# jinhan/tacotron2-vae

Measured on AMD Instinct MI355X. Metric: mel-frames/s (train step, batch=6, 80-mel), higher is better.
Workload: dtype f32; 1 GPU; configs[1]: Tacotron2-VAE fp32 train step (fwd+loss+bwd+clip+Adam), B=6/GPU fixed shape T_in=84 T_out=400, dropout on, random-init seed 1234; step_mode=hip-graph replay, decoder_forward=persistent, decoder_backward=persistent, startup_steps=43, global_batch=6, parallelism=dp1

## Files before the change

include/t2vae.h:

```cpp
#ifndef T2VAE_H
#define T2VAE_H
#include <stdint.h>
#ifdef __cplusplus
extern "C" {
#endif

#define T2V_OK 0
#define T2V_ERR_DIMS -1
#define T2V_ERR_ARG -2
#define T2V_ERR_LAUNCH -3

const char* t2v_version(void);
const char* t2v_last_error(void);

void t2v_set_phase_profile(unsigned long long* dev_buf32);
int t2v_stamp(unsigned long long* dev_buf, int slot, void* stream);
int t2v_debug_spin(int wgs, int microseconds, void* stream);

typedef struct t2v_step_params {
    uint64_t epoch;
    float lr;
    float bc1;
    float bc2s;
    float kl_weight;
// ... 223 lines not shown

int t2v_bn_act_fwd(const float* y, const float* stat_part, int nblk, const float* gamma, const float* beta,
                   float* running_mean, float* running_var, float* mean_out, float* rstd_out, float* out,
                   int B, int M, int T, int act, int training, float p_drop, float momentum, float eps,
                   uint64_t seed, uint32_t rng_stream, uint32_t rng_t, void* stream);
int t2v_bn_act_fwd_len(const float* y, const float* gamma, const float* beta, const float* running_mean,
                       const float* running_var, float* out, const int32_t* lengths, int B, int M, int T, int act, float eps,
                       void* stream);
int t2v_bn_act_bwd(const float* y, const float* dout, const float* mean, const float* rstd,
                   const float* gamma, const float* beta, float* dy, float* dgamma, float* dbeta,
                   float* dconv_bias, int B, int M, int T, int act, float p_drop, uint64_t seed,
                   uint32_t rng_stream, uint32_t rng_t, void* stream);
int t2v_bn_act_bwd_eval(const float* y, const float* dout, const float* mean, const float* rstd,
                   const float* gamma, const float* beta, float* dy, float* dgamma, float* dbeta,
                   float* dconv_bias, int B, int M, int T, int act, float p_drop, uint64_t seed,
                   uint32_t rng_stream, uint32_t rng_t, void* stream);

int t2v_embedding_fwd(const long long* ids, const float* W, float* out_bct, int B, int T, int C, int n_symbols, void* stream);
int t2v_embedding_bwd(const long long* ids, const float* dy_bct, float* dW, int B, int T, int C, int n_symbols, void* stream);

int t2v_gemm_epilogue_bwd(const float* dy, const float* y, float* out, size_t n, float scale, void* stream);

long t2v_colsum_scratch_floats(long M, long N);
int t2v_colsum(const float* A, long lda, long M, long N, float* scratch, float* out, void* stream);

int t2v_mask_outputs(float* mel, float* mel_post, float* gate, const int* lengths, int B, int C, int T, float gate_fill,
                     void* stream);
int t2v_mask_time(const float* x, float* out, const int32_t* lengths, int B, int C, int T, void* stream);
int t2v_reparam_fwd(const float* eps, const float* mu, const float* logvar, float* z, long n, void* stream);
int t2v_reparam_bwd(const float* dz, const float* eps, const float* logvar, float* dlogvar, long n, void* stream);
int t2v_gather_words(const void* const* src, void* const* dst, int n, void* stream);
int t2v_concat2_rows(const float* a, long lda, int na, const float* b, long ldb, int nb, float* out, long rows, void* stream);

int t2v_bilstm_fwd(const float* gx, const float* whh, const int32_t* lengths, float* y, float* gates,
                   float* cells, float* hx_scratch, uint32_t* sync3, int B, int T, void* stream);
int t2v_bilstm_bwd(const float* whh, const int32_t* lengths, const float* dy, const float* gates,
                   const float* cells, float* dg, float* dgx_scratch, uint32_t* sync3, int B, int T,
                   void* stream);

int t2v_gemm_f32(const float* A, long sAi, long sAk, const float* B, long sBj, long sBk, const float* bias,
                 float* C, int ldc, int M, int N, int K, int relu, int accumulate, float p_drop,
                 uint64_t seed, uint32_t rng_stream, uint32_t rng_t, void* stream);
long t2v_gemm_splitk_scratch_floats(int M, int N, int K);
int t2v_gemm_f32_splitk(const float* A, long sAi, long sAk, const float* B, long sBj, long sBk, const float* bias,
                        float* C, int ldc, int M, int N, int K, int relu, int accumulate, float p_drop,
                        uint64_t seed, uint32_t rng_stream, uint32_t rng_t, float* splitk_scratch, void* stream);

int t2v_gemm_f32_set_mode(int x3);

typedef struct t2v_gemm_group {
    const float* A;
    long sAi;
    long sAk;
    int nb;
    const float* B[3];
    long sBj[3];
    long sBk[3];
    int N[3];
    float* C[3];
    int ldc[3];
} t2v_gemm_group;
long t2v_gemm_f32_grouped_scratch_floats(const t2v_gemm_group* groups, int ngroups, int M, int K);
int t2v_gemm_f32_grouped(const t2v_gemm_group* groups, int ngroups, int M, int K, int accumulate, float* scratch, void* stream);
long t2v_gemm_f32_grouped_group_offset(const t2v_gemm_group* groups, int ngroups, int M, int K, int g);
int t2v_gemm_f32_grouped_handed(const t2v_gemm_group* groups, int ngroups, int M, int K, int accumulate, float* scratch, int handed,
                                const uint32_t* done_ctr, int done_cap, void* stream);
// ... 160 lines not shown
```

tacotron2-vae_amd/csrc/gemm.hip:

```cpp
#include <stdlib.h>
#include <string.h>
#include "t2v_common.h"
#include "t2v_kernels.h"
#include "t2v_coop.h"
#include "t2v_x3.h"
#include "t2v_xchg.h"
#include "gemm_x3_tile.h"

#define GM_BM 64
#define GM_BN 64
#define GM_BK 32

struct GemmArgs {
    const float* A; const float* B; const float* bias; float* C;
    long sAi, sAk, sBj, sBk;
    int M, N, K, ldc;
    int relu, accumulate;
    float p_drop; uint64_t seed; uint32_t rng_stream, rng_t;
    const t2v_step_params* step;
    int kz_chunk;
    float* part;
    int nbatch;
    long sAb, sBb, sCb;
    int nsub;
// ... 137 lines not shown
                || hipDeviceSynchronize() != hipSuccess) { state.store(0); return nullptr; }
            ring = p;
            state.store(2, std::memory_order_release);
        } else {
            while (state.load(std::memory_order_acquire) == 1) { }
            if (state.load() != 2) return nullptr;
        }
    }
    unsigned at = pos.fetch_add((unsigned)tiles);
    at %= GM_CTR_RING;
    if (at + (unsigned)tiles > GM_CTR_RING) {
        pos.store((unsigned)tiles);
        at = 0;
    }
    return ring + at;
}
static int gemm_splits(int M, int N, int K) {
    const long tiles = (long)((M + GM_BM - 1) / GM_BM) * ((N + GM_BN - 1) / GM_BN);
    static const int wide = getenv("T2V_GEMM_SPLIT_POLICY") ? atoi(getenv("T2V_GEMM_SPLIT_POLICY")) : 1;
    if (wide) {
        if (tiles > 256 || K < 8 * GM_BK) return 1;
        long ns2 = (512 + tiles - 1) / tiles;
        const long maxk2 = K / (4 * GM_BK);
        if (ns2 > maxk2) ns2 = maxk2;
        if (ns2 > 32) ns2 = 32;
        return ns2 < 2 ? 1 : (int)ns2;
    }
    if (tiles >= 256 || K < 16 * GM_BK) return 1;
    long ns = 512 / tiles;
    const long maxk = K / (8 * GM_BK);
    if (ns > maxk) ns = maxk;
    if (ns > 32) ns = 32;
    return ns < 2 ? 1 : (int)ns;
}
static bool gemm_x3_shape_ok(int M, int N, int K);
static long gemm_x3_scratch_floats(int M, int N, int K, int np);
static int gemm_x3_mode();
extern "C" long t2v_gemm_splitk_scratch_floats(int M, int N, int K) {
    if (M < 1 || N < 1 || K < 1) return 0;
    if (gemm_x3_mode() && gemm_x3_shape_ok(M, N, K)) return gemm_x3_scratch_floats(M, N, K, 3);
    const int ns = gemm_splits(M, N, K);
    return ns > 1 ? (long)ns * M * N : 0;
}

#define GB_BM 128
#define GB_BK 32
#define GB_LD 160
template <bool A_KC, bool B_KC, int BN>
__global__ __launch_bounds__(256) void k_gemm_f32_big(GemmArgs a) {
    constexpr int NY = BN / 64;
    constexpr int NA = GB_BM * GB_BK / 4 / 256;
    constexpr int NB = BN * GB_BK / 4 / 256;
    constexpr int KQ = GB_BK / 4;
    __shared__ __attribute__((aligned(16))) float As[2][GB_BK][GB_LD];
    __shared__ __attribute__((aligned(16))) float Bs[2][GB_BK][BN + 32];
    const int tid = threadIdx.x, wave = tid >> 6, lane = tid & 63;
    const int wm = wave >> 1, wn = wave & 1;
    int by_ = blockIdx.y, bx_ = blockIdx.x;
    {
        const int nb = gridDim.x * gridDim.y, bid = blockIdx.y * gridDim.x + blockIdx.x;
        const int q = nb >> 3, r = nb & 7, xcd = bid & 7, idx = bid >> 3;
        const int lin = (xcd < r ? xcd * (q + 1) : r * (q + 1) + (xcd - r) * q) + idx;
        by_ = lin / gridDim.x;
        bx_ = lin - by_ * gridDim.x;
    }
    const int i0 = by_ * GB_BM, j0 = bx_ * BN;
// ... 796 lines not shown
```

tacotron2-vae_amd/csrc/t2v_kernels.h:

```cpp
#pragma once
#include <hip/hip_runtime.h>
#include <stdint.h>
#include <initializer_list>
#include "../../include/t2vae.h"
#include "t2v_common.h"

enum { T2V_RNG_ATT_H = 1, T2V_RNG_ATT_C = 2, T2V_RNG_DEC_H = 3, T2V_RNG_DEC_C = 4,
       T2V_RNG_PRENET0 = 5, T2V_RNG_PRENET1 = 6 };

int t2v_check_launch();
unsigned* t2v_arrival_counters(int n);
extern unsigned long long* g_t2v_prof;
const t2v_step_params* t2v_step_for(hipStream_t stream);

struct T2VZeroRegions {
    void* p[10];
    size_t bytes[10];
    int n = 0;
    void add(void* ptr, size_t nbytes) { p[n] = ptr; bytes[n] = nbytes; ++n; }
};
void t2v_zero_regions(T2VZeroRegions& z, hipStream_t stream);

__global__ void k_sentinel_fill(uint4* p, size_t n16);
void t2v_fill_sentinel(void* p, size_t n16, int grid, hipStream_t stream);
bool t2v_persist_cus_ok();
bool t2v_persist_raise_lds(std::initializer_list<const void*> kernels, bool& raised);
int t2v_persist_resident(const void* kernel, int threads, size_t lds, std::initializer_list<const void*> kernels, bool& raised);
struct LstmFwdArgs;
struct AttnFwdArgs;

typedef unsigned long long t2v_u64;
static inline size_t t2v_tcap(int T_in) { return (size_t)((T_in + 15) / 16) * 16; }
static inline size_t t2v_qp_sync_off(int B) { return (size_t)B * 256 * 128; }
static inline size_t t2v_qp_xchg_off(int B) { return t2v_qp_sync_off(B) + 64; }
static inline size_t t2v_qp_ex_off(int B) { return t2v_qp_sync_off(B) + 64 + 4096; }
#define T2V_MAX_T_IN 4096
static inline size_t t2v_qp_floats(int B, int T_in) { return t2v_qp_ex_off(B) + 2 * (size_t)B * 8 * t2v_tcap(T_in); }
static inline int t2v_attn_bwd_js(int T_in) { return T_in <= 128 ? 16 : 32; }
static inline int t2v_attn_bwd_slices_(int T_in) { const int js = t2v_attn_bwd_js(T_in); return (T_in + js - 1) / js; }
void t2v_launch_lstm_fwd(int mode, const LstmFwdArgs& a, hipStream_t stream);
void t2v_launch_attn_fwd(const AttnFwdArgs& f, int B, int T_in, hipStream_t stream);
void t2v_launch_attn_fwd_window(const AttnFwdArgs& f, int B, int T_in, int back, int ahead, hipStream_t stream);
static inline unsigned* t2v_persist_fwd_begin(const t2v_dec_train_persist_weights* w, const t2v_dec_train_bufs* s, const float* scratch,
                                              int B, int T_in, hipStream_t stream) {
// ... 129 lines not shown
```

tacotron2-vae_amd/model.py:

```python
from math import sqrt

import os

import torch
from torch import nn
from torch.nn import functional as F

import t2v_hip
from layers import ConvNorm, LinearNorm
from modules import VAE_GST
from utils import get_mask_from_lengths, to_gpu

drop_rate = 0.5
_drop_seed = [0x5EED]


class LocationLayer(nn.Module):
    def __init__(self, attention_n_filters, attention_kernel_size, attention_dim):
        super().__init__()
        self.location_conv = ConvNorm(2, attention_n_filters, kernel_size=attention_kernel_size,
                                      padding=(attention_kernel_size - 1) // 2, bias=False, stride=1,
                                      dilation=1)
        self.location_dense = LinearNorm(attention_n_filters, attention_dim, bias=False, w_init_gain='tanh')

# ... 335 lines not shown
        dec = self.decoder_rnn
        return (dec.bias_ih + dec.bias_hh,
                torch.cat((self.linear_projection.weight, self.gate_layer.weight), 0),
                torch.cat((self.linear_projection.bias, self.gate_layer.bias), 0))

    def forward(self, memory, decoder_inputs, memory_lengths):
        B, T_in = memory.size(0), memory.size(1)
        prep = self.__dict__.pop('_prepared', None)
        gpre = None
        operands = None
        if prep is not None and prep[0] is decoder_inputs:
            _, pre, gpre, st, operands = prep
            T = pre.size(0)
            if st != torch.cuda.current_stream():
                torch.cuda.current_stream().wait_stream(st)
                for t in operands:
                    t.record_stream(torch.cuda.current_stream())
        else:
            frames = self.parse_decoder_inputs(decoder_inputs)
            T = frames.size(0)
            x = torch.cat((self.get_go_frame(memory).unsqueeze(0), frames), 0)
            pre = self.prenet(x[:T], self._tf_rng_t())
        att = self.attention_rnn
        lin = t2v_hip.LinearHIP.apply
        pm = lin(memory, self.attention_layer.memory_layer.weight, None, False, 0.0, 0, 0, 0)
        lengths = lengths_i32(memory_lengths, memory.device)
        training = self.training
        p_att = self.p_attention_dropout if training else 0.0
        p_dec = self.p_decoder_dropout if training else 0.0
        self._calls += 1
        seed = (int(self.dropout_seed) * 1000003 + self._calls) & 0x7FFFFFFFFFFFFFFF
        t2v_hip.stamp('dec_fwd_begin')
        b_dec, w81, b81 = operands if operands is not None else self._param_operands()
        hc, alignments = t2v_hip.DecoderCore.apply(None, memory, pm, lengths, *self._core_weights(b_dec),
                                                   p_att, p_dec, seed, torch.is_grad_enabled(),
                                                   pre, att.bias_ih, att.bias_hh, gpre)
        t2v_hip.stamp('dec_fwd_end')
        out = lin(hc, w81, b81, False, 0.0, 0, 0, 0)
        mel = out[..., :self.n_mel_channels].permute(1, 2, 0).contiguous()
        gate = out[..., self.n_mel_channels].transpose(0, 1).contiguous()
        return mel, gate, alignments


class SymbolEmbedding(nn.Embedding):

    def forward(self, ids):
        return t2v_hip.SymbolEmbedding.apply(ids, self.weight)


def lengths_i32(lengths, device):
    v = getattr(lengths, '_i32', None)
    if v is not None and v.device == device:
        return v
    return lengths.to(device=device, dtype=torch.int32)


class BatchLayout(object):
    _DT = (torch.int64, torch.int64, torch.float32, torch.float32, torch.int64, torch.float32, torch.float32)
    _ring = {}
    RING = 4
    n_symbols = None

    @classmethod
    def check_ids(cls, text):
        if cls.n_symbols is not None and text.numel() and not text.is_cuda:
            lo, hi = int(text.min()), int(text.max())
            if lo < 0 or hi >= cls.n_symbols:
                raise IndexError("symbol id out of range: got [%d, %d], embedding has %d rows" % (lo, hi, cls.n_symbols))

# ... 160 lines not shown
```

tacotron2-vae_amd/t2v_hip.py:

```python
import collections
import ctypes as C
import math
import operator
import os

import torch

_HERE = os.path.dirname(os.path.abspath(__file__))
_LIB_PATH = os.environ.get('T2V_LIB') or os.path.join(_HERE, 'libt2vae_hip.so')
_lib = None

H, E, PRE, A, F_LOC, KS, XW, KATT, KATT_INF, G4 = 1024, 512, 256, 128, 32, 31, 2560, 1536, 1792, 4096


class T2VHipError(RuntimeError):
    pass


class _DecWeights(C.Structure):
    _fields_ = [(n, C.c_void_p) for n in (
        'packF_att', 'packF_dec', 'packB_att', 'packB_dec', 'bias_att', 'bias_dec', 'wqT', 'wcomb', 'v')] + [
        ('packs_bf16', C.c_int32)]


# ... 52 lines not shown
    _fields_ = [('back', C.c_int32), ('ahead', C.c_int32)]


EXPORTS = ('t2v_version', 't2v_last_error', 't2v_stamp', 't2v_debug_spin', 't2v_pack_lstm_weights', 't2v_pack_lstm_weights_bf16', 't2v_decoder_train_fwd',
           't2v_decoder_train_bwd', 't2v_clip_adam_step', 't2v_clip_adam_step_guarded', 't2v_decoder_replay_fwd_kernels', 't2v_mel_frontend', 't2v_set_phase_profile', 't2v_decoder_infer_steps', 't2v_conv1d_stat_blocks', 't2v_conv1d_stat_blocks_bf16', 't2v_conv1d_staged_launches', 't2v_conv1d_fwd', 't2v_conv1d_bwd', 't2v_conv1d_fwd_bf16', 't2v_conv1d_bwd_bf16', 't2v_conv1d_dw_scratch_floats', 't2v_conv1d_flip_weights', 't2v_gemm_bf16', 't2v_gemm_bf16_splitk', 't2v_gemm_bf16_splitk_scratch_floats', 't2v_attn_wgrad', 't2v_attn_wgrad_scratch_floats',
           't2v_bn_act_fwd', 't2v_bn_act_bwd', 't2v_bn_act_bwd_eval', 't2v_bilstm_fwd', 't2v_bilstm_bwd', 't2v_gemm_f32', 't2v_conv2d_s2_fwd', 't2v_conv2d_s2_bwd', 't2v_conv2d_s2_dw_scratch_floats', 't2v_conv2d_s2_fwd_gemm', 't2v_conv2d_s2_bwd_gemm',
           't2v_conv2d_s2_gemm_scratch_floats',
           't2v_gru_fwd', 't2v_gru_bwd', 't2v_loss_fwd_bwd', 't2v_fuse_location_weights', 't2v_decoder_qp_floats',
           't2v_set_step_params', 't2v_set_step_params_stream', 't2v_decoder_replay_bwd_kernels', 't2v_embedding_fwd', 't2v_embedding_bwd', 't2v_gemm_f32_splitk', 't2v_gemm_splitk_scratch_floats', 't2v_gemm_f32_batched',
           't2v_decoder_infer_persistent', 't2v_decoder_persist_supported', 't2v_decoder_persist_scratch_floats',
           't2v_attn_bwd_slices', 't2v_colsum', 't2v_colsum_scratch_floats', 't2v_gemm_epilogue_bwd',
           't2v_decoder_train_fwd_persistent', 't2v_decoder_train_persist_supported',
           't2v_decoder_train_persist_scratch_floats', 't2v_decoder_bwd_persist_supported',
           't2v_decoder_bwd_achain_scratch_floats', 't2v_decoder_bwd_achain', 't2v_decoder_bwd_achain_prepare',
           't2v_decoder_bwd_achain_prepared', 't2v_decoder_bwd_persist_slices', 't2v_decoder_bwd_achain_dq_offset',
           't2v_decoder_bwd_achain_dw_offset', 't2v_gemm_f32_grouped_handed', 't2v_gemm_f32_grouped_group_offset', 't2v_mask_outputs', 't2v_reparam_fwd',
           't2v_reparam_bwd', 't2v_gather_words', 't2v_concat2_rows',
           't2v_decoder_train_fwd_persistent16', 't2v_decoder_train_persist16_supported',
           't2v_decoder_train_persist16_scratch_floats', 't2v_decoder_bwd_persistent16', 't2v_decoder_bwd_persist16_supported',
           't2v_decoder_bwd_persist16_scratch_floats', 't2v_decoder_bwd_persist16_dq_offset', 't2v_decoder_bwd_persist16_slices',
           't2v_decoder_bwd_persist16_fits', 't2v_gemm_f32_set_mode', 't2v_conv1d_x3_set_mode', 't2v_gemm_f32_grouped',
           't2v_gemm_f32_grouped_scratch_floats', 't2v_gemm_bf16_grouped', 't2v_gemm_bf16_grouped_scratch_floats',
           't2v_decoder_bwd_persistent16_prepare', 't2v_decoder_bwd_persistent16_prepared',
           't2v_stft_polar', 't2v_istft', 't2v_istft_scratch_bytes', 't2v_griffin_lim', 't2v_griffin_lim_scratch_bytes',
           't2v_mel_to_magnitude', 't2v_decoder_infer_steps_items', 't2v_decoder_infer_persistent_items', 't2v_bn_act_fwd_len',
           't2v_mask_time', 't2v_conv2d_s2_fwd_ragged', 't2v_conv2d_s2_fwd_gemm_ragged', 't2v_conv2d_s2_gemm_ragged_scratch_floats',
           't2v_gru_fwd_len', 't2v_mel_dtw', 't2v_mel_dtw_scratch_bytes', 't2v_tsne_scratch_bytes', 't2v_tsne_affinities',
           't2v_tsne_gradient', 't2v_tsne_run', 't2v_f0_yin', 't2v_alignment_stats', 't2v_alignment_scratch_bytes',
           't2v_mel_to_magnitude_nnls', 't2v_griffin_lim_fast', 't2v_griffin_lim_fast_scratch_bytes',
           't2v_resample', 't2v_trim_bounds', 't2v_crop_rows', 't2v_latent_scratch_bytes', 't2v_latent_neighbours',
           't2v_mel_cepstrum', 't2v_cep_dtw_scratch_bytes', 't2v_cep_dtw_path', 't2v_cep_dtw_forward', 't2v_cep_dtw_walk',
           't2v_path_scores', 't2v_loudness', 't2v_loudness_scratch_bytes', 't2v_scale_rows',
           't2v_decoder_infer_steps_window', 't2v_decoder_infer_persistent_window',
           't2v_phase_vocoder', 't2v_phase_vocoder_scratch_bytes')


def lib_path():
    return _LIB_PATH


def load_library():
    global _lib
    if _lib is not None:
        return _lib
    if not os.path.isfile(_LIB_PATH):
        raise T2VHipError("libt2vae_hip.so not built: run `python -c 'import __graft_entry__ as g; g.build()'` "
                          "(or make -C tacotron2-vae_amd/csrc)")
    lib = C.CDLL(_LIB_PATH)
    lib.t2v_version.restype = C.c_char_p
    lib.t2v_last_error.restype = C.c_char_p
    lib.t2v_pack_lstm_weights.argtypes = [C.c_void_p, C.c_void_p, C.c_void_p, C.c_void_p, C.c_int, C.c_void_p,
                                          C.c_void_p, C.c_void_p, C.c_void_p, C.c_void_p]
    lib.t2v_pack_lstm_weights_bf16.argtypes = [C.c_void_p, C.c_void_p, C.c_void_p, C.c_void_p, C.c_int, C.c_void_p,
                                          C.c_void_p, C.c_void_p, C.c_void_p, C.c_void_p]
    lib.t2v_fuse_location_weights.argtypes = [C.c_void_p, C.c_void_p, C.c_void_p, C.c_void_p]
    lib.t2v_decoder_qp_floats.argtypes = [C.c_int, C.c_int]
    lib.t2v_decoder_qp_floats.restype = C.c_long
    lib.t2v_attn_bwd_slices.argtypes = [C.c_int]
    lib.t2v_decoder_train_fwd.argtypes = [C.POINTER(_DecWeights), C.POINTER(_DecTrainBufs), C.c_int, C.c_int,
                                          C.c_int, C.c_float, C.c_float, C.c_uint64, C.c_void_p]
    lib.t2v_decoder_train_bwd.argtypes = [C.POINTER(_DecWeights), C.POINTER(_DecTrainBufs),
                                          C.POINTER(_DecBwdBufs), C.c_int, C.c_int, C.c_int, C.c_float,
                                          C.c_float, C.c_uint64, C.c_void_p]
    lib.t2v_decoder_train_fwd_persistent.argtypes = [C.POINTER(_DecTrainPersistWeights), C.POINTER(_DecTrainBufs), C.c_void_p,
                                                     C.c_int, C.c_int, C.c_int, C.c_float, C.c_float, C.c_uint64, C.c_void_p]
    lib.t2v_decoder_train_persist_supported.argtypes = [C.c_int, C.c_int]
    lib.t2v_decoder_train_fwd_persistent16.argtypes = lib.t2v_decoder_train_fwd_persistent.argtypes
# ... 22 lines not shown
    lib.t2v_decoder_train_persist_scratch_floats.argtypes = [C.c_int, C.c_int, C.c_int]
    lib.t2v_decoder_train_persist_scratch_floats.restype = C.c_long
    lib.t2v_decoder_bwd_persist_supported.argtypes = [C.c_int, C.c_int]
    lib.t2v_decoder_bwd_achain_scratch_floats.argtypes = [C.c_int, C.c_int, C.c_int]
    lib.t2v_decoder_bwd_achain_scratch_floats.restype = C.c_long
    lib.t2v_gemm_f32_grouped_handed.argtypes = [C.POINTER(_GemmGroup), C.c_int, C.c_int, C.c_int, C.c_int, C.c_void_p, C.c_int, C.c_void_p,
                                                C.c_int, C.c_void_p]
    lib.t2v_gemm_f32_grouped_group_offset.argtypes = [C.POINTER(_GemmGroup), C.c_int, C.c_int, C.c_int, C.c_int]
    lib.t2v_gemm_f32_grouped_group_offset.restype = C.c_long
    lib.t2v_decoder_bwd_achain_dw_offset.argtypes = [C.c_int, C.c_int, C.c_int]
    lib.t2v_decoder_bwd_achain_dw_offset.restype = C.c_long
    lib.t2v_decoder_bwd_achain.argtypes = [C.POINTER(_DecTrainPersistWeights), C.POINTER(_AchainDw), C.POINTER(_DecTrainBufs)] + [C.c_void_p] * 8 + [
        C.c_int, C.c_int, C.c_int, C.c_float, C.c_float, C.c_uint64, C.c_void_p]
    lib.t2v_decoder_bwd_persist_slices.argtypes = [C.c_int]
    lib.t2v_decoder_bwd_achain_dq_offset.argtypes = [C.c_int, C.c_int, C.c_int]
    lib.t2v_decoder_bwd_achain_dq_offset.restype = C.c_long
    lib.t2v_decoder_bwd_achain_prepared.argtypes = lib.t2v_decoder_bwd_achain.argtypes
    lib.t2v_decoder_bwd_achain_prepare.argtypes = [C.POINTER(_DecTrainBufs), C.c_void_p, C.c_void_p, C.c_void_p, C.c_int, C.c_int, C.c_int,
                                                   C.c_float, C.c_float, C.c_uint64, C.c_void_p]
    lib.t2v_decoder_replay_fwd_kernels.argtypes = [C.POINTER(_DecWeights), C.POINTER(_DecTrainBufs), C.c_int,
                                                   C.c_int, C.c_int, C.c_float, C.c_float, C.c_uint64, C.c_int,
                                                   C.c_void_p]
    lib.t2v_decoder_replay_bwd_kernels.argtypes = [C.POINTER(_DecWeights), C.POINTER(_DecTrainBufs),
                                                   C.POINTER(_DecBwdBufs), C.c_int, C.c_int, C.c_int, C.c_float,
                                                   C.c_float, C.c_uint64, C.c_int, C.c_void_p]
    lib.t2v_clip_adam_step.argtypes = [C.c_void_p, C.c_void_p, C.c_void_p, C.c_void_p, C.c_uint64, C.c_float,
                                       C.c_float, C.c_float, C.c_float, C.c_float, C.c_float, C.c_float,
                                       C.c_float, C.c_float, C.c_void_p, C.c_void_p, C.c_void_p]
    lib.t2v_clip_adam_step_guarded.argtypes = lib.t2v_clip_adam_step.argtypes[:-1] + [C.c_void_p, C.c_int, C.c_void_p]
    lib.t2v_mask_outputs.argtypes = [C.c_void_p] * 4 + [C.c_int, C.c_int, C.c_int, C.c_float, C.c_void_p]
    lib.t2v_reparam_fwd.argtypes = [C.c_void_p] * 4 + [C.c_long, C.c_void_p]
    lib.t2v_reparam_bwd.argtypes = [C.c_void_p] * 4 + [C.c_long, C.c_void_p]
    lib.t2v_concat2_rows.argtypes = [C.c_void_p, C.c_long, C.c_int, C.c_void_p, C.c_long, C.c_int, C.c_void_p, C.c_long, C.c_void_p]
    lib.t2v_gather_words.argtypes = [C.POINTER(C.c_void_p), C.POINTER(C.c_void_p), C.c_int, C.c_void_p]
    lib.t2v_embedding_fwd.argtypes = [C.c_void_p, C.c_void_p, C.c_void_p, C.c_int, C.c_int, C.c_int, C.c_int, C.c_void_p]
    lib.t2v_embedding_bwd.argtypes = [C.c_void_p, C.c_void_p, C.c_void_p, C.c_int, C.c_int, C.c_int, C.c_int, C.c_void_p]
    lib.t2v_gemm_epilogue_bwd.argtypes = [C.c_void_p, C.c_void_p, C.c_void_p, C.c_size_t, C.c_float, C.c_void_p]
    lib.t2v_colsum.argtypes = [C.c_void_p, C.c_long, C.c_long, C.c_long, C.c_void_p, C.c_void_p, C.c_void_p]
    lib.t2v_colsum_scratch_floats.argtypes = [C.c_long, C.c_long]
    lib.t2v_colsum_scratch_floats.restype = C.c_long
    lib.t2v_set_step_params.argtypes = [C.c_void_p]
    lib.t2v_set_step_params.restype = None
    lib.t2v_set_step_params_stream.argtypes = [C.c_void_p, C.c_void_p]
    lib.t2v_mel_frontend.argtypes = [C.c_void_p, C.c_void_p, C.c_void_p, C.c_int, C.c_int, C.c_float, C.c_int,
                                     C.c_int, C.c_int, C.c_void_p, C.c_void_p, C.c_void_p, C.c_void_p, C.c_void_p,
                                     C.c_void_p, C.c_int, C.c_void_p, C.c_int, C.c_void_p]
    lib.t2v_set_phase_profile.argtypes = [C.c_void_p]
    lib.t2v_set_phase_profile.restype = None
    lib.t2v_stamp.argtypes = [C.c_void_p, C.c_int, C.c_void_p]
    lib.t2v_debug_spin.argtypes = [C.c_int, C.c_int, C.c_void_p]
    lib.t2v_decoder_infer_persistent.argtypes = [C.POINTER(_DecPersistWeights), C.POINTER(_DecPersistBufs), C.c_int, C.c_int,
                                                 C.c_int, C.c_float, C.c_float, C.c_uint64, C.c_void_p]
    lib.t2v_decoder_infer_persistent_items.argtypes = lib.t2v_decoder_infer_persistent.argtypes[:-1] + [C.POINTER(_DecItems),
                                                                                                        C.c_void_p]
    lib.t2v_decoder_persist_supported.argtypes = [C.c_int, C.c_int]
    lib.t2v_decoder_persist_scratch_floats.argtypes = [C.c_int, C.c_int]
    lib.t2v_decoder_persist_scratch_floats.restype = C.c_long
    lib.t2v_decoder_infer_steps.argtypes = [C.POINTER(_DecWeights), C.POINTER(_DecInferBufs), C.c_int, C.c_int, C.c_int,
                                            C.c_int, C.c_float, C.c_float, C.c_int, C.c_uint64, C.c_void_p]
    lib.t2v_decoder_infer_steps_items.argtypes = lib.t2v_decoder_infer_steps.argtypes[:-1] + [C.POINTER(_DecItems), C.c_void_p]
    lib.t2v_decoder_infer_steps_window.argtypes = lib.t2v_decoder_infer_steps_items.argtypes[:-1] + [C.POINTER(_DecWindow), C.c_void_p]
    lib.t2v_decoder_infer_persistent_window.argtypes = lib.t2v_decoder_infer_persistent_items.argtypes[:-1] + [C.POINTER(_DecWindow),
                                                                                                               C.c_void_p]
    vp = C.c_void_p
    lib.t2v_stft_polar.argtypes = [vp, vp, C.c_int, C.c_int, C.c_int, C.c_int, vp, vp, vp, vp, vp, C.c_int, vp]
    lib.t2v_istft_scratch_bytes.argtypes = [C.c_int, C.c_int]
# ... 654 lines not shown
    _check(load_library().t2v_decoder_replay_bwd_kernels(C.byref(W), C.byref(Sb), C.byref(Gb), B, T_in, T, p_att, p_dec,
                                                         seed, int(kernel_mask), _stream()),
           't2v_decoder_replay_bwd_kernels')
    return T if kernel_mask == 1 else T + 1


def pack_decoder_weights(w_ih_att, w_hh_att, w_ih_dec, w_hh_dec, k_att, need_bwd, bf16=False, need_fwd=True):
    lib = load_library()
    dev = w_ih_att.device
    f32 = dict(device=dev, dtype=torch.float32)
    w_ih_att, w_hh_att, w_ih_dec, w_hh_dec = (_f32c(t.detach()) for t in (w_ih_att, w_hh_att, w_ih_dec, w_hh_dec))
    need_fwd = need_fwd or not need_bwd
    packF_att = torch.empty(G4 * k_att, **f32) if need_fwd else None
    packF_dec = torch.empty(G4 * XW, **f32) if need_fwd else None
    packB_att = torch.empty(G4 * KATT, **f32) if need_bwd else None
    packB_dec = torch.empty(G4 * XW, **f32) if need_bwd else None
    fn = lib.t2v_pack_lstm_weights_bf16 if bf16 else lib.t2v_pack_lstm_weights
    _check(fn(_p(w_ih_att), _p(w_hh_att), _p(w_ih_dec), _p(w_hh_dec), int(k_att),
              _p(packF_att), _p(packF_dec), _p(packB_att), _p(packB_dec), _stream()), 't2v_pack_lstm_weights')
    return packF_att, packF_dec, packB_att, packB_dec


def fuse_location_weights(loc_conv, loc_dense):
    lib = load_library()
    wcomb = torch.empty(2, A, 64, device=loc_conv.device, dtype=torch.float32)
    _check(lib.t2v_fuse_location_weights(_p(loc_conv), _p(loc_dense), _p(wcomb), _stream()), 't2v_fuse_location_weights')
    return wcomb


class DecoderCore(torch.autograd.Function):
    persistent = None
    persistent_bwd = None
    persistent16 = None
    keep_last = False
    last_call = None
    last_persist = None
    last_bwd = None
    last_bwd_persist = None
    last_persist_engine = last_bwd_persist_engine = None
    dw_tile_cap = None
    last_mode = None
    last_bwd_mode = None
    last_kernel = None
    last_bwd_kernel = None
    chunk_kernels = []
    chunk_bwd_kernels = []

    @staticmethod
    def plan(lib, B, T_in, T, need_grad):
        D = DecoderCore
        env = os.environ.get
        fwd_on = D.persistent if D.persistent is not None else env('T2V_TRAIN_PERSISTENT', '1') != '0'
        bwd_on = D.persistent_bwd if D.persistent_bwd is not None else env('T2V_BWD_PERSISTENT', env('T2V_TRAIN_PERSISTENT', '1')) != '0'
        on16 = D.persistent16 if D.persistent16 is not None else env('T2V_PERSIST16', '1') != '0'
        force = on16 == 'force'
        on16 = bool(on16) and bool(_BF16)
        small = lambda floats: 4 * floats < 2 ** 31 - 1
        chunks = [(b0, min(B, b0 + MAX_DEC_B)) for b0 in range(0, B, MAX_DEC_B)]
        fwd, bwd = [], []
        for b0, b1 in chunks:
            b = b1 - b0
            p32 = bool(fwd_on) and bool(lib.t2v_decoder_train_persist_supported(b, T_in)) and \
                small(lib.t2v_decoder_train_persist_scratch_floats(b, T_in, T))
            f16 = on16 and bool(fwd_on) and bool(lib.t2v_decoder_train_persist16_supported(b, T_in)) and (force or not p32) and \
                small(lib.t2v_decoder_train_persist16_scratch_floats(b, T_in, T))
            fwd.append('persist16' if f16 else 'persist' if p32 else 'steps')
            if need_grad:
                r32 = bool(bwd_on) and bool(lib.t2v_decoder_bwd_persist_supported(b, T_in)) and \
                    small(lib.t2v_decoder_bwd_achain_scratch_floats(b, T_in, T))
                r16 = on16 and env('T2V_PERSIST16_BWD', '1') != '0' and bool(bwd_on) and \
                    bool(lib.t2v_decoder_bwd_persist16_fits(b, T_in, T)) and (force or not r32)
                bwd.append('persist16' if r16 else 'achain' if r32 else 'steps')
            else:
                bwd.append(None)
        if 'steps' in bwd:
            bwd = ['steps'] * len(bwd)
        dw_on = (not _BF16 and env('T2V_DW_EPILOGUE', '1') != '0' and env('T2V_DW_GROUPED', '1') != '0' and
                 env('T2V_F32_GEMM', '') not in ('native', '0'))
        return [ChunkPlan(b0, b1, f, r, f != 'steps' and r in _BWD_ENGINES, dw_on and r == 'achain')
                for (b0, b1), f, r in zip(chunks, fwd, bwd)]

    @staticmethod
    def _note(fwd=None, bwd=None, **kept):
        D = DecoderCore
        if fwd is not None:
            D.last_mode = 'launch-per-step' if fwd == 'steps' else 'persistent'
            D.last_kernel = _STEPS_KERNELS['fwd'] if fwd == 'steps' else _FWD_ENGINES[fwd].kernel
            D.chunk_kernels.append(D.last_kernel)
        if bwd is not None:
            D.last_bwd_mode = 'launch-per-step' if bwd == 'steps' else 'persistent'
            D.last_bwd_kernel = _STEPS_KERNELS['bwd'] if bwd == 'steps' else _BWD_ENGINES[bwd].kernel
            D.chunk_bwd_kernels.append(D.last_bwd_kernel)
        for name, value in kept.items():
            setattr(D, name, value)

    @staticmethod
    def _wgrad_tensors(ctx, f32):
        if ctx.wg is None:
            wg = [grad_slot(w) for w in ctx.wrefs]
            ctx.wg = [torch.empty(w.shape, **f32) if g is None else g for g, w in zip(wg, ctx.wrefs)]
        return ctx.wg

    @staticmethod
    def _dw_groups(DGA, DGD, XS, wg, pre_c, T, B):
        TB = T * B
        x_prev, x_cur = XS[0:T].reshape(TB, XW), XS[1:T + 1].reshape(TB, XW)
        d_w_ih_att, d_w_hh_att, d_w_ih_dec, d_w_hh_dec = wg
        att = [(x_prev[:, :H].t(), d_w_hh_att), (x_prev[:, H:KATT].t(), d_w_ih_att[:, PRE:])]
        if pre_c is not None:
            att.insert(0, (pre_c.t(), d_w_ih_att[:, :PRE]))
        return [(DGA.view(TB, G4).t(), att), (DGD.view(TB, G4).t(), [(x_cur[:, :KATT].t(), d_w_ih_dec), (x_cur[:, KATT:].t(), d_w_hh_dec)])]

    @staticmethod
# ... 20 lines not shown
        keep = (gpre, memory, pm, lengths, XS, CA, CD, GA, GD, QP, AL, ACUM, S)
        packF_att, packF_dec, packB_att, packB_dec = packs
        W = _DecWeights(_p(packF_att), _p(packF_dec), _p(packB_att), _p(packB_dec), None, _p(bias_dec),
                        _p(wqT), _p(wcomb), _p(vv), int(bool(wbf)))
        Sb = _DecTrainBufs(*(_p(t) for t in keep))
        dims = (B, T_in, T, float(p_att), float(p_dec), int(seed))
        if plan.fwd == 'steps':
            _check(lib.t2v_decoder_train_fwd(C.byref(W), C.byref(Sb), *(dims + (_stream(),))), 't2v_decoder_train_fwd')
            _err_note('decoder forward (attention exchange)', QP.view(torch.int32)[B * 256 * A + 31:][:1])
            DecoderCore._note(fwd='steps')
            return W, Sb, keep, None
        eng = _FWD_ENGINES[plan.fwd]
        scratch = torch.empty(getattr(lib, eng.scratch)(B, T_in, T), **f32)
        PW = _persist_weights(raw, bias_dec, wcomb, vv)
        _check(getattr(lib, eng.run)(C.byref(PW), C.byref(Sb), _p(scratch), *(dims + (_stream(),))), eng.run)
        _err_note('decoder forward (persistent kernel hand-off)', QP.view(torch.int32)[B * 256 * A + 31:][:1])
        DecoderCore._note(fwd=plan.fwd)
        if DecoderCore.keep_last:
            DecoderCore._note(last_persist=(PW, Sb, scratch, dims, raw), last_persist_engine=plan.fwd)
        if not plan.prepare:
            return W, Sb, keep, None
        beng = _BWD_ENGINES[plan.bwd]
        DQP, bscr, errw = DecoderCore._bwd_buffers(lib, beng, B, T_in, T, gpre.device)
        with side('w', keep=tuple(keep[_ARENA.index(n)] for n in beng.keep)):
            args = (_p(DQP), _p(bscr), _p(errw), B, T_in, T)
            if beng.arena_prepare:
                args = (C.byref(Sb),) + args + dims[3:]
            _check(getattr(lib, beng.prepare)(*(args + (_stream(),))), beng.prepare)
            ev = torch.cuda.Event()
            ev.record()
        return W, Sb, keep, (DQP, bscr, errw, ev)

    @staticmethod
    def forward(ctx, gpre, memory, pm, lengths, w_ih_att, w_hh_att, w_ih_dec, w_hh_dec, bias_dec,
                wq, loc_conv, loc_dense, v, p_att, p_dec, seed, grad_mode=True, pre=None, b_ih_att=None, b_hh_att=None,
                gpre_ready=None):
        lib = _require_gpu(memory, pm, w_ih_att)
        pre2 = None
        if pre is not None:
            assert gpre is None
            pre2 = _f32c(pre).view(-1, PRE)
            if gpre_ready is not None:
                gpre = gpre_ready.view(pre.shape[0], pre.shape[1], G4)
            else:
                gpre = gemm(pre2, w_ih_att.detach()[:, :PRE], (b_ih_att + b_hh_att).detach()).view(pre.shape[0], pre.shape[1], G4)
        T, B, _ = gpre.shape
        T_in = memory.shape[1]
        gpre, memory, pm = _f32c(gpre), _f32c(memory), _f32c(pm)
        need_grad = bool(grad_mode) and any(ctx.needs_input_grad)
        wbf = bool(_BF16)
        plans = DecoderCore.plan(lib, B, T_in, T, need_grad)
        fwd_persist = all(p.fwd != 'steps' for p in plans)
        bwd_persist = need_grad and all(p.bwd != 'steps' for p in plans)
        if fwd_persist and (bwd_persist or not need_grad):
            packs = (None, None, None, None)
        else:
            packs = pack_decoder_weights(w_ih_att, w_hh_att, w_ih_dec, w_hh_dec, KATT, need_grad and not bwd_persist, bf16=wbf,
                                         need_fwd=not fwd_persist)
        raw = tuple(_f32c(t.detach()) for t in (w_ih_att, w_hh_att, w_ih_dec, w_hh_dec, wq))
        wqT = wq.detach().t().contiguous()
        bias_dec = _f32c(bias_dec.detach())
        loc_conv, loc_dense, vv = _f32c(loc_conv.detach()), _f32c(loc_dense.detach()), _f32c(v.detach()).view(-1)
        wcomb = fuse_location_weights(loc_conv, loc_dense)
        chunks = []
        DecoderCore._note(chunk_kernels=[])
        for p in plans:
            if p.b0 == 0 and p.b1 == B:
                g_c, m_c, pm_c, l_c = gpre, memory, pm, lengths
            else:
                g_c, m_c, pm_c = gpre[:, p.b0:p.b1].contiguous(), memory[p.b0:p.b1].contiguous(), pm[p.b0:p.b1].contiguous()
                l_c = None if lengths is None else lengths[p.b0:p.b1].contiguous()
            chunks.append(DecoderCore._fwd_chunk(lib, p, g_c, m_c, pm_c, l_c, packs, bias_dec, wqT, wcomb, vv, need_grad,
                                                 p_att, p_dec, _chunk_seed(seed, p.b0), wbf, raw))
        hcs = []
        for _w, _s, k, _prep in chunks:
            XSc = k[4]
            Bc, XWc = XSc.size(1), XSc.size(2)
            hc_c = torch.empty(T, Bc, XWc - H, device=XSc.device, dtype=torch.float32)
            _check(lib.t2v_concat2_rows(_p(XSc[2:, :, KATT:]), XWc, XWc - KATT, _p(XSc[1:, :, H:KATT]), XWc, KATT - H, _p(hc_c),
                                        T * Bc, _stream()), 't2v_concat2_rows')
            hcs.append(hc_c)
        als = [k[10][1:].permute(1, 0, 2) for _, _, k, _ in chunks]
        HC, align = _cat(hcs, 1), _cat(als, 0)
        ctx.dims = (B, T_in, T, float(p_att), float(p_dec), int(seed))
        ctx.consts = (packs, bias_dec, wqT, wcomb, vv, loc_conv, loc_dense)
        ctx.wbf = wbf
        ctx.wrefs = (w_ih_att, w_hh_att, w_ih_dec, w_hh_dec)
        ctx.raw = raw
        ctx.pre2 = pre2
        ctx.pre_on_side = gpre_ready is not None
        ctx.plans = plans
        ctx.chunks = [k for _, _, k, _ in chunks] if need_grad else None
        ctx.prepared = [pr for _, _, _, pr in chunks] if need_grad else None
        ctx.mark_non_differentiable(align)
        if DecoderCore.keep_last:
            W0, S0, k0, _ = chunks[0]
            DecoderCore._note(last_call=(W0, S0, (k0[0].shape[1], T_in, T, float(p_att), float(p_dec), int(seed)),
                                         k0 + (packs, bias_dec, wqT, wcomb, vv)))
        return HC, align

    @staticmethod
    def _pre_chunk(ctx, b0, B):
        Bt, _, T = ctx.dims[:3]
        return ctx.pre2 if ctx.pre2 is None or B == Bt else ctx.pre2.view(T, Bt, PRE)[:, b0:b0 + B].reshape(T * B, PRE)

    @staticmethod
    def _bwd_persist(ctx, lib, ci, dhc_c, DGA, DGD, DCTX):
        plan, keep, b0, B = ctx.plans[ci], ctx.chunks[ci], ctx.plans[ci].b0, DGA.size(1)
        _, T_in, T, p_att, p_dec, seed = ctx.dims
        _packs, bias_dec, _wqT, wcomb, vv = ctx.consts[:5]
        eng = _BWD_ENGINES[plan.bwd]
        f32 = dict(device=dhc_c.device, dtype=torch.float32)
        DV = torch.empty(B, getattr(lib, eng.slices)(T_in), A, **f32)
        Sb = _DecTrainBufs(*(_p(t) for t in keep))
        PW = _persist_weights(ctx.raw, bias_dec, wcomb, vv)
        prep, ctx.prepared[ci] = ctx.prepared[ci], None
        if prep is not None:
            DQP, scratch, errw, pev = prep
            torch.cuda.current_stream().wait_event(pev)
        else:
            DQP, scratch, errw = DecoderCore._bwd_buffers(lib, eng, B, T_in, T, dhc_c.device)
        dwh = None
        if plan.dw_epilogue and set_f32_gemm_mode(None) and T * B >= 32:
            groups = DecoderCore._dw_groups(DGA, DGD, keep[4], DecoderCore._wgrad_tensors(ctx, f32), DecoderCore._pre_chunk(ctx, b0, B), T, B)
            dwh = GroupedHandOver(groups, 1, scratch[lib.t2v_decoder_bwd_achain_dw_offset(B, T_in, T):][:1], ci > 0, DecoderCore.dw_tile_cap)
            if ci > 0 and overlap() is not None:
                overlap().wait('g')
        stamp('dec_bwd_begin')
        bufs = (dhc_c, DGA, DGD, DCTX, DV, DQP, scratch, errw)
        _bwd_launch(lib, eng, prep is not None, PW, Sb, bufs, (B, T_in, T, p_att, p_dec, _chunk_seed(seed, b0)),
                    None if dwh is None else dwh.dw)
        _err_note('decoder backward (persistent kernel hand-off)', errw)
# ... 86 lines not shown
    def backward(ctx, dHC, _dalign):
        lib = load_library()
        if ctx.chunks is None:
            raise T2VHipError("DecoderCore.backward without a saved arena (forward ran under no_grad)")
        Bt, _T_in, T = ctx.dims[:3]
        f32 = dict(device=dHC.device, dtype=torch.float32)
        dHC = _f32c(dHC)
        acc = bacc = ctx.wg = None
        dga_l, dmem_l, dpm_l, dpre_l = [], [], [], []
        DecoderCore._note(chunk_bwd_kernels=[])
        for ci, plan in enumerate(ctx.plans):
            b0, B = plan.b0, plan.b1 - plan.b0
            dhc_c = dHC if B == Bt else dHC[:, b0:b0 + B].contiguous()
            DGA, DGD, DCTX = torch.empty(T, B, G4, **f32), torch.empty(T, B, G4, **f32), torch.empty(T, B, E, **f32)
            reverse = DecoderCore._bwd_persist if plan.bwd in _BWD_ENGINES else DecoderCore._bwd_steps
            rev = reverse(ctx, lib, ci, dhc_c, DGA, DGD, DCTX)
            d_memory, d_pm, acc, bparts = DecoderCore._chunk_grads(ctx, lib, ci, dhc_c, DGA, DGD, DCTX, *rev, acc, dpre_l)
            bacc = bparts if bacc is None else [x + y for x, y in zip(bacc, bparts)]
            dmem_l.append(d_memory); dpm_l.append(d_pm); dga_l.append(DGA)
        ctx.chunks = ctx.prepared = None
        wg, ctx.wg = ctx.wg, None
        d_memory, d_pm = _cat(dmem_l, 0), _cat(dpm_l, 0)
        DGA = d_pre = d_b_att = None
        if ctx.pre2 is not None:
            d_b_att = bacc[1]
            if dpre_l and ctx.pre_on_side:
                with side('w'):
                    d_pre = _cat(dpre_l, 1)
            elif dpre_l:
                d_pre = _cat(dpre_l, 1)
        else:
            DGA = _cat(dga_l, 1)
        return (DGA, d_memory, d_pm, None, *wg, bacc[0], *acc, None, None, None, None, d_pre, d_b_att, d_b_att, None)


def attn_wgrad(dpre, AL, ACUM, loc_conv, loc_dense, B, T_in, T):
    lib = _require_gpu(dpre, AL, ACUM, loc_conv, loc_dense)
    f32 = dict(device=dpre.device, dtype=torch.float32)
    part = torch.empty(lib.t2v_attn_wgrad_scratch_floats(), **f32)
    d_dense, d_conv = torch.empty(A, F_LOC, **f32), torch.empty(F_LOC, 2, KS, **f32)
    _check(lib.t2v_attn_wgrad(_p(dpre), _p(AL), _p(ACUM), _p(_f32c(loc_conv)), _p(_f32c(loc_dense)), _p(part),
                              _p(d_dense), _p(d_conv), B, T_in, T, _stream()), 't2v_attn_wgrad')
    return d_dense, d_conv


def mel_frontend(wav, n_samples, tables, scale=1.0, t_stride=None):
    lib = _require_gpu(wav)
    B, N = wav.shape
    wav = wav.contiguous()
    if int(n_samples.min()) <= 512 or int(n_samples.max()) > N:
        raise ValueError("mel_frontend: every utterance needs 512 < n_samples <= %d, got [%d, %d]"
                         % (N, int(n_samples.min()), int(n_samples.max())))
    n_samples = n_samples.to(device=wav.device, dtype=torch.int64).contiguous()
    if t_stride is None:
        t_stride = int(n_samples.max().item()) // 256 + 1
    out = torch.empty(B, 80, t_stride, device=wav.device, dtype=torch.float32)
    is16 = wav.dtype == torch.int16
    if not is16 and wav.dtype != torch.float32:
        raise T2VHipError("mel_frontend takes float32 or int16 samples")
    _check(lib.t2v_mel_frontend(None if is16 else _p(wav), _p(wav) if is16 else None, _p(n_samples), B, N,
                                float(scale), 1024, 256, 80, _p(tables['window']), _p(tables['tw512']),
                                _p(tables['tw1024']), _p(tables['mel_start']), _p(tables['mel_len']),
                                _p(tables['mel_w']), int(tables['maxw']), _p(out), t_stride, _stream()),
           't2v_mel_frontend')
    return out

# ... 1717 lines not shown
```

Before: 230,900 mel-frames/s.

## Fuse decoder output projection into a head kernel reading the arena directly

Adds a fused head kernel that reads hidden/context rows straight from the decoder arena and applies the 81-wide mel+gate projection. It writes mel and gate in their final [B,C,T] layout, replacing the concat, GEMM, slice and permute-contiguous ops. The backward uses a pack kernel to transpose dmel/dgate into the GEMM layout and computes the weight gradients on a side stream, overlapping them with the decoder backward. The forward matches the old split-K summation order via a k-chunk, and the backward still gathers hc for the weight gradient.

```diff
diff --git a/include/t2vae.h b/include/t2vae.h
--- a/include/t2vae.h
+++ b/include/t2vae.h
@@ -279,6 +279,10 @@
 int t2v_gather_words(const void* const* src, void* const* dst, int n, void* stream);
 int t2v_concat2_rows(const float* a, long lda, int na, const float* b, long ldb, int nb, float* out, long rows, void* stream);
 
+int t2v_head_fwd(const float* a, long lda, int na, const float* b, long ldb, int nb, const float* W, const float* bias,
+                 float* mel, float* gate, int B, int T, int Btot, void* stream);
+int t2v_head_bwd_pack(const float* dmel, const float* dgate, float* dy, int B, int T, void* stream);
+
 int t2v_bilstm_fwd(const float* gx, const float* whh, const int32_t* lengths, float* y, float* gates,
                    float* cells, float* hx_scratch, uint32_t* sync3, int B, int T, void* stream);
 int t2v_bilstm_bwd(const float* whh, const int32_t* lengths, const float* dy, const float* gates,
diff --git a/tacotron2-vae_amd/csrc/gemm.hip b/tacotron2-vae_amd/csrc/gemm.hip
--- a/tacotron2-vae_amd/csrc/gemm.hip
+++ b/tacotron2-vae_amd/csrc/gemm.hip
@@ -193,6 +193,10 @@
     if (ns > maxk) ns = maxk;
     if (ns > 32) ns = 32;
     return ns < 2 ? 1 : (int)ns;
+}
+int t2v_gemm64_k_chunk(int M, int N, int K) {
+    const int ns = gemm_splits(M, N, K);
+    return ns > 1 ? ((K + GM_BK - 1) / GM_BK + ns - 1) / ns * GM_BK : 0;
 }
 static bool gemm_x3_shape_ok(int M, int N, int K);
 static long gemm_x3_scratch_floats(int M, int N, int K, int np);
diff --git a/tacotron2-vae_amd/csrc/head.hip b/tacotron2-vae_amd/csrc/head.hip
--- /dev/null
+++ b/tacotron2-vae_amd/csrc/head.hip
@@ -0,0 +1,121 @@
+#include "t2v_common.h"
+#include "t2v_kernels.h"
+
+#define HD_N (T2V_NMEL + 1)
+#define HD_NT 6
+#define HD_TT 16
+#define HD_KS 32
+#define HD_WAVES 8
+#define HD_ROWS (HD_TT + 16 * HD_NT)
+#define HD_LD (HD_KS + 4)
+
+__global__ __launch_bounds__(64 * HD_WAVES) void k_head_fwd(const float* __restrict__ a, long lda, int na, const float* __restrict__ b,
+                                                            long ldb, int nb, const float* __restrict__ W, const float* __restrict__ bias,
+                                                            float* __restrict__ mel, float* __restrict__ gate, int B, int T, int kchunk) {
+    const int tid = threadIdx.x, lane = tid & 63, wave = tid >> 6;
+    const int item = blockIdx.y, t0 = blockIdx.x * HD_TT;
+    const int K = na + nb, nst = K / HD_KS, nst_a = na / HD_KS;
+    __shared__ __attribute__((aligned(16))) float tile[2][HD_ROWS][HD_LD];
+
+    const int c = tid & 7, r0 = tid >> 3;
+    const long xrow = (long)min(t0 + r0, T - 1) * B + item;
+    const float* px_a = a + xrow * lda + 4 * c;
+    const float* px_b = b + xrow * ldb + 4 * c;
+    auto wrow = [&](int r) { return W + (size_t)min(max(r - HD_TT, 0), HD_N - 1) * K + 4 * c; };
+    const float *pw0 = wrow(r0), *pw1 = wrow(r0 + 64);
+    const bool frame = wave < 2, two = wave < 6;
+    float4 st0, st1;
+    auto gload = [&](int s) {
+        if (frame) st0 = s < nst_a ? *(const float4*)(px_a + s * HD_KS) : *(const float4*)(px_b + (s - nst_a) * HD_KS);
+        else st0 = *(const float4*)(pw0 + s * HD_KS);
+        if (two) st1 = *(const float4*)(pw1 + s * HD_KS);
+    };
+    auto sstore = [&](int buf) {
+        *(float4*)&tile[buf][r0][4 * c] = st0;
+        if (two) *(float4*)&tile[buf][r0 + 64][4 * c] = st1;
+    };
+
+    const int rl = lane & 15, g = lane >> 4, nt = wave;
+    f32x4 acc = {0.f, 0.f, 0.f, 0.f}, sum = {0.f, 0.f, 0.f, 0.f};
+    auto mma = [&](int buf, int s) {
+        if (nt < HD_NT) {
+            float x[HD_KS / 4], w[HD_KS / 4];
+#pragma unroll
+            for (int q = 0; q < HD_KS / 4; ++q) {
+                x[q] = tile[buf][rl][4 * q + g];
+                w[q] = tile[buf][HD_TT + 16 * nt + rl][4 * q + g];
+            }
+#pragma unroll
+            for (int q = 0; q < HD_KS / 4; ++q) acc = mfma16x4(w[q], x[q], acc);
+            if (kchunk && (((s + 1) * HD_KS) % kchunk == 0 || s + 1 == nst)) {
+                sum += acc;
+                acc = f32x4{0.f, 0.f, 0.f, 0.f};
+            }
+        }
+    };
+
+    gload(0);
+    sstore(0);
+    __syncthreads();
+    for (int s = 0; s < nst; s += 2) {
+        if (s + 1 < nst) gload(s + 1);
+        mma(0, s);
+        if (s + 1 >= nst) break;
+        sstore(1);
+        __syncthreads();
+        if (s + 2 < nst) gload(s + 2);
+        mma(1, s + 1);
+        if (s + 2 < nst) sstore(0);
+        __syncthreads();
+    }
+    if (nt >= HD_NT) return;
+    if (!kchunk) sum = acc;
+    const int t = t0 + rl;
+#pragma unroll
+    for (int r = 0; r < 4; ++r) {
+        const int n = 16 * nt + 4 * g + r;
+        if (n >= HD_N || t >= T) continue;
+        const float v = sum[r] + bias[n];
+        if (n < T2V_NMEL) mel[((size_t)item * T2V_NMEL + n) * T + t] = v;
+        else gate[(size_t)item * T + t] = v;
+    }
+}
+
+extern "C" int t2v_head_fwd(const float* a, long lda, int na, const float* b, long ldb, int nb, const float* W, const float* bias,
+                            float* mel, float* gate, int B, int T, int Btot, void* stream_) {
+    if (!a || !b || !W || !bias || !mel || !gate || B < 1 || T < 1 || B > 65535 || Btot < B || (long)T * Btot > 0x7fffffff ||
+        na < 0 || nb < 0 || na + nb < HD_KS || ((na | nb) & (HD_KS - 1)) || ((lda | ldb) & 3) || lda < na || ldb < nb ||
+        (((uintptr_t)a | (uintptr_t)b | (uintptr_t)W) & 15))
+        return T2V_ERR_ARG;
+    const dim3 grid((unsigned)((T + HD_TT - 1) / HD_TT), (unsigned)B);
+    const int kchunk = t2v_gemm64_k_chunk(T * Btot, HD_N, na + nb);
+    k_head_fwd<<<grid, 64 * HD_WAVES, 0, (hipStream_t)stream_>>>(a, lda, na, b, ldb, nb, W, bias, mel, gate, B, T, kchunk);
+    return t2v_check_launch();
+}
+
+#define HP_TT 32
+
+__global__ __launch_bounds__(256) void k_head_bwd_pack(const float* __restrict__ dmel, const float* __restrict__ dgate, float* __restrict__ dy,
+                                                       int B, int T) {
+    const int tid = threadIdx.x, item = blockIdx.y, t0 = blockIdx.x * HP_TT;
+    const int nt = min(HP_TT, T - t0);
+    __shared__ float tile[HD_N][HP_TT + 1];
+    const int tl = tid & (HP_TT - 1);
+    for (int n = tid / HP_TT; n < HD_N; n += 256 / HP_TT) {
+        float v = 0.f;
+        if (tl < nt) v = n < T2V_NMEL ? dmel[((size_t)item * T2V_NMEL + n) * T + t0 + tl] : dgate[(size_t)item * T + t0 + tl];
+        tile[n][tl] = v;
+    }
+    __syncthreads();
+    for (int i = tid; i < nt * HD_N; i += 256) {
+        const int fl = i / HD_N, n = i - fl * HD_N;
+        dy[((size_t)(t0 + fl) * B + item) * HD_N + n] = tile[n][fl];
+    }
+}
+
+extern "C" int t2v_head_bwd_pack(const float* dmel, const float* dgate, float* dy, int B, int T, void* stream_) {
+    if (!dmel || !dgate || !dy || B < 1 || T < 1 || B > 65535) return T2V_ERR_ARG;
+    const dim3 grid((unsigned)((T + HP_TT - 1) / HP_TT), (unsigned)B);
+    k_head_bwd_pack<<<grid, 256, 0, (hipStream_t)stream_>>>(dmel, dgate, dy, B, T);
+    return t2v_check_launch();
+}
diff --git a/tacotron2-vae_amd/csrc/t2v_kernels.h b/tacotron2-vae_amd/csrc/t2v_kernels.h
--- a/tacotron2-vae_amd/csrc/t2v_kernels.h
+++ b/tacotron2-vae_amd/csrc/t2v_kernels.h
@@ -10,6 +10,7 @@
 
 int t2v_check_launch();
 unsigned* t2v_arrival_counters(int n);
+int t2v_gemm64_k_chunk(int M, int N, int K);
 extern unsigned long long* g_t2v_prof;
 const t2v_step_params* t2v_step_for(hipStream_t stream);
 
diff --git a/tacotron2-vae_amd/model.py b/tacotron2-vae_amd/model.py
--- a/tacotron2-vae_amd/model.py
+++ b/tacotron2-vae_amd/model.py
@@ -391,9 +391,11 @@
         seed = (int(self.dropout_seed) * 1000003 + self._calls) & 0x7FFFFFFFFFFFFFFF
         t2v_hip.stamp('dec_fwd_begin')
         b_dec, w81, b81 = operands if operands is not None else self._param_operands()
-        hc, alignments = t2v_hip.DecoderCore.apply(None, memory, pm, lengths, *self._core_weights(b_dec),
-                                                   p_att, p_dec, seed, torch.is_grad_enabled(),
-                                                   pre, att.bias_ih, att.bias_hh, gpre)
+        core = (None, memory, pm, lengths, *self._core_weights(b_dec), p_att, p_dec, seed, torch.is_grad_enabled(),
+                pre, att.bias_ih, att.bias_hh, gpre)
+        if t2v_hip.DecoderCore.use_fused_head():
+            return t2v_hip.DecoderHeadCore.apply(*core, w81, b81)
+        hc, alignments = t2v_hip.DecoderCore.apply(*core)
         t2v_hip.stamp('dec_fwd_end')
         out = lin(hc, w81, b81, False, 0.0, 0, 0, 0)
         mel = out[..., :self.n_mel_channels].permute(1, 2, 0).contiguous()
diff --git a/tacotron2-vae_amd/t2v_hip.py b/tacotron2-vae_amd/t2v_hip.py
--- a/tacotron2-vae_amd/t2v_hip.py
+++ b/tacotron2-vae_amd/t2v_hip.py
@@ -108,7 +108,8 @@
            't2v_mel_cepstrum', 't2v_cep_dtw_scratch_bytes', 't2v_cep_dtw_path', 't2v_cep_dtw_forward', 't2v_cep_dtw_walk',
            't2v_path_scores', 't2v_loudness', 't2v_loudness_scratch_bytes', 't2v_scale_rows',
            't2v_decoder_infer_steps_window', 't2v_decoder_infer_persistent_window',
-           't2v_phase_vocoder', 't2v_phase_vocoder_scratch_bytes')
+           't2v_phase_vocoder', 't2v_phase_vocoder_scratch_bytes',
+           't2v_head_fwd', 't2v_head_bwd_pack')
 
 
 def lib_path():
@@ -197,6 +198,8 @@
     lib.t2v_reparam_fwd.argtypes = [C.c_void_p] * 4 + [C.c_long, C.c_void_p]
     lib.t2v_reparam_bwd.argtypes = [C.c_void_p] * 4 + [C.c_long, C.c_void_p]
     lib.t2v_concat2_rows.argtypes = [C.c_void_p, C.c_long, C.c_int, C.c_void_p, C.c_long, C.c_int, C.c_void_p, C.c_long, C.c_void_p]
+    lib.t2v_head_fwd.argtypes = [C.c_void_p, C.c_long, C.c_int, C.c_void_p, C.c_long, C.c_int] + [C.c_void_p] * 4 + [C.c_int] * 3 + [C.c_void_p]
+    lib.t2v_head_bwd_pack.argtypes = [C.c_void_p] * 3 + [C.c_int, C.c_int, C.c_void_p]
     lib.t2v_gather_words.argtypes = [C.POINTER(C.c_void_p), C.POINTER(C.c_void_p), C.c_int, C.c_void_p]
     lib.t2v_embedding_fwd.argtypes = [C.c_void_p, C.c_void_p, C.c_void_p, C.c_int, C.c_int, C.c_int, C.c_int, C.c_void_p]
     lib.t2v_embedding_bwd.argtypes = [C.c_void_p, C.c_void_p, C.c_void_p, C.c_int, C.c_int, C.c_int, C.c_int, C.c_void_p]
@@ -917,6 +920,7 @@
     persistent = None
     persistent_bwd = None
     persistent16 = None
+    fused_head = None
     keep_last = False
     last_call = None
     last_persist = None
@@ -964,6 +968,12 @@
                  env('T2V_F32_GEMM', '') not in ('native', '0'))
         return [ChunkPlan(b0, b1, f, r, f != 'steps' and r in _BWD_ENGINES, dw_on and r == 'achain')
                 for (b0, b1), f, r in zip(chunks, fwd, bwd)]
+
+    @staticmethod
+    def use_fused_head():
+        D = DecoderCore
+        on = D.fused_head if D.fused_head is not None else os.environ.get('T2V_FUSED_HEAD', '1') != '0'
+        return bool(on) and not _BF16
 
     @staticmethod
     def _note(fwd=None, bwd=None, **kept):
@@ -1050,9 +1060,13 @@
         return W, Sb, keep, (DQP, bscr, errw, ev)
 
     @staticmethod
-    def forward(ctx, gpre, memory, pm, lengths, w_ih_att, w_hh_att, w_ih_dec, w_hh_dec, bias_dec,
-                wq, loc_conv, loc_dense, v, p_att, p_dec, seed, grad_mode=True, pre=None, b_ih_att=None, b_hh_att=None,
-                gpre_ready=None):
+    def forward(ctx, *args):
+        return DecoderCore._forward(ctx, None, *args)
+
+    @staticmethod
+    def _forward(ctx, head, gpre, memory, pm, lengths, w_ih_att, w_hh_att, w_ih_dec, w_hh_dec, bias_dec,
+                 wq, loc_conv, loc_dense, v, p_att, p_dec, seed, grad_mode=True, pre=None, b_ih_att=None, b_hh_att=None,
+                 gpre_ready=None):
         lib = _require_gpu(memory, pm, w_ih_att)
         pre2 = None
         if pre is not None:
@@ -1090,16 +1104,13 @@
                 l_c = None if lengths is None else lengths[p.b0:p.b1].contiguous()
             chunks.append(DecoderCore._fwd_chunk(lib, p, g_c, m_c, pm_c, l_c, packs, bias_dec, wqT, wcomb, vv, need_grad,
                                                  p_att, p_dec, _chunk_seed(seed, p.b0), wbf, raw))
-        hcs = []
-        for _w, _s, k, _prep in chunks:
-            XSc = k[4]
-            Bc, XWc = XSc.size(1), XSc.size(2)
-            hc_c = torch.empty(T, Bc, XWc - H, device=XSc.device, dtype=torch.float32)
-            _check(lib.t2v_concat2_rows(_p(XSc[2:, :, KATT:]), XWc, XWc - KATT, _p(XSc[1:, :, H:KATT]), XWc, KATT - H, _p(hc_c),
-                                        T * Bc, _stream()), 't2v_concat2_rows')
-            hcs.append(hc_c)
+        if head is None:
+            out = (gather_hc([k[4] for _, _, k, _ in chunks], T),)
+        else:
+            stamp('dec_fwd_end')
+            out = head_fwd([k[4] for _, _, k, _ in chunks], [p.b0 for p in plans], head[0], head[1], B, T)
         als = [k[10][1:].permute(1, 0, 2) for _, _, k, _ in chunks]
-        HC, align = _cat(hcs, 1), _cat(als, 0)
+        align = _cat(als, 0)
         ctx.dims = (B, T_in, T, float(p_att), float(p_dec), int(seed))
         ctx.consts = (packs, bias_dec, wqT, wcomb, vv, loc_conv, loc_dense)
         ctx.wbf = wbf
@@ -1115,7 +1126,7 @@
             W0, S0, k0, _ = chunks[0]
             DecoderCore._note(last_call=(W0, S0, (k0[0].shape[1], T_in, T, float(p_att), float(p_dec), int(seed)),
                                          k0 + (packs, bias_dec, wqT, wcomb, vv)))
-        return HC, align
+        return out + (align,)
 
     @staticmethod
     def _pre_chunk(ctx, b0, B):
@@ -1268,6 +1279,82 @@
         else:
             DGA = _cat(dga_l, 1)
         return (DGA, d_memory, d_pm, None, *wg, bacc[0], *acc, None, None, None, None, d_pre, d_b_att, d_b_att, None)
+
+
+def _arena_hc(XS, T):
+    TB = T * XS.size(1)
+    return XS[2:T + 2].reshape(TB, XW)[:, KATT:], XS[1:T + 1].reshape(TB, XW)[:, H:KATT]
+
+
+def gather_hc(arenas, T):
+    lib = _require_gpu(*arenas)
+    hcs = []
+    for XS in arenas:
+        hd, cx = _arena_hc(XS, T)
+        hc_c = torch.empty(T, XS.size(1), XW - H, device=XS.device, dtype=torch.float32)
+        _check(lib.t2v_concat2_rows(_p(hd), XW, hd.size(1), _p(cx), XW, cx.size(1), _p(hc_c), T * XS.size(1), _stream()),
+               't2v_concat2_rows')
+        hcs.append(hc_c)
+    return _cat(hcs, 1)
+
+
+def head_fwd(arenas, b0s, w81, b81, B, T, mel=None, gate=None):
+    lib = _require_gpu(w81, b81, *arenas)
+    N = w81.shape[0] - 1
+    w81, b81 = _f32c(w81.detach()), _f32c(b81.detach())
+    f32 = dict(device=w81.device, dtype=torch.float32)
+    mel = torch.empty(B, N, T, **f32) if mel is None else mel
+    gate = torch.empty(B, T, **f32) if gate is None else gate
+    for XS, b0 in zip(arenas, b0s):
+        assert XS.is_contiguous() and XS.size(2) == XW and XS.size(0) >= T + 2 and 0 <= b0 and b0 + XS.size(1) <= B
+        assert mel.is_contiguous() and gate.is_contiguous() and mel.shape[1:] == (N, T) and gate.shape[1:] == (T,)
+        hd, cx = _arena_hc(XS, T)
+        _check(lib.t2v_head_fwd(_p(hd), XW, hd.size(1), _p(cx), XW, cx.size(1), _p(w81), _p(b81), _p(mel[b0:]), _p(gate[b0:]),
+                                XS.size(1), T, B, _stream()), 't2v_head_fwd')
+    return mel, gate
+
+
+def head_bwd_pack(dmel, dgate):
+    lib = _require_gpu(dmel, dgate)
+    dmel, dgate = _f32c(dmel), _f32c(dgate)
+    B, N, T = dmel.shape
+    assert dgate.shape == (B, T)
+    dy2 = torch.empty(T * B, N + 1, device=dmel.device, dtype=torch.float32)
+    _check(lib.t2v_head_bwd_pack(_p(dmel), _p(dgate), _p(dy2), B, T, _stream()), 't2v_head_bwd_pack')
+    return dy2
+
+
+class DecoderHeadCore(torch.autograd.Function):
+
+    @staticmethod
+    def forward(ctx, *args):
+        w81, b81 = args[-2:]
+        out = DecoderCore._forward(ctx, (w81, b81), *args[:-2])
+        ctx.w81 = _f32c(w81.detach())
+        return out
+
+    @staticmethod
+    def backward(ctx, dmel, dgate, _dalign):
+        if ctx.chunks is None:
+            raise T2VHipError("DecoderHeadCore.backward without a saved arena (forward ran under no_grad)")
+        B, _T_in, T = ctx.dims[:3]
+        dy2 = head_bwd_pack(dmel, dgate)
+        fork = mark()
+        dHC = gemm(dy2, ctx.w81.t()).view(T, B, XW - H)
+        arenas = [k[4] for k in ctx.chunks]
+        ev = None
+        with side('w', keep=(dy2,) + tuple(arenas), after=fork) as forked:
+            dw81 = gemm(dy2.t(), gather_hc(arenas, T).view(T * B, XW - H).t())
+            db81 = colsum(dy2)
+            if forked:
+                ev = torch.cuda.Event()
+                ev.record()
+        core = DecoderCore.backward(ctx, dHC, None)
+        if ev is not None:
+            torch.cuda.current_stream().wait_event(ev)
+            for g in (dw81, db81):
+                g.record_stream(torch.cuda.current_stream())
+        return core + (dw81, db81)
 
 
 def attn_wgrad(dpre, AL, ACUM, loc_conv, loc_dense, B, T_in, T):
```

New measurement: 233,100 mel-frames/s (median of 6 runs). No clear change (+1.0%).
